# ucsdarclab/Python-SuPer

Hardware: AMD Instinct MI355X
Metric: LM iterations/s (embedded-deformation LM, point-to-plane + ARAP + Rot) (higher is better)
Workload: dtype f64; 1 GPU; C2: 200000 surfels / 2000 ED nodes / KNN=4, point-to-plane + ARAP + Rot, 10 LM iterations + Surfels.update per frame; frames_per_gpu=8, streams_per_gpu=1, global_frames=8, parallelism=frames sharded over 1 GPU(s), beta all-gather

## Files before the change

python-super_amd/csrc/slm_api.hip:

```cpp
#include <new>
#include <cstdio>

#include "slm_solver.h"

static thread_local std::string g_err;

void slm_set_error_text(const char* msg) { g_err = msg; }

std::atomic<long long> g_reallocs{0}, g_realloc_bytes{0}, g_plan_builds{0}, g_plan_reuses{0}, g_plan_fill_hits{0};

int check_slots(slm_solver* s, int first, int n) {
  if (!s) return fail(SLM_ERR_INVALID, "null solver");
  if (first < 0 || n < 1 || first + n > (int)s->slots.size())
    return fail(SLM_ERR_INVALID, "slot range out of bounds");
  for (int i = first; i < first + n; ++i) {
    join_prepare(s, i);
    if (!s->slots[i].h.bound) return fail(SLM_ERR_UNBOUND, "slot used before slm_bind_frame");
    if (s->slots[i].h.f.K != s->slots[first].h.f.K)
      return fail(SLM_ERR_UNSUPPORTED, "the frames of one batch must have the same num_neighbors");
  }
  return SLM_OK;
}

extern "C" {
// ... 120 lines not shown
  }
  return SLM_OK;
}

int slm_device_count(void) {
  int n = 0;
  if (hipGetDeviceCount(&n) != hipSuccess) return 0;
  return n;
}

int slm_create(const slm_config* cfg, slm_solver** out) {
  if (!cfg || !out) return fail(SLM_ERR_INVALID, "slm_create: null argument");
  if (cfg->max_frames < 1 || cfg->num_iterations < 0 || !(cfg->v > 0.0))
    return fail(SLM_ERR_INVALID, "slm_create: bad config");
  if (cfg->solver_path < 0 || cfg->solver_path > 4) return fail(SLM_ERR_INVALID, "slm_create: solver_path must be 0..4");
  if (cfg->data_path < 0 || cfg->data_path > 2) return fail(SLM_ERR_INVALID, "slm_create: data_path must be 0..2");
  if (slm_device_count() < 1) return fail(SLM_ERR_NO_DEVICE, "slm_create: no HIP device visible");
  slm_solver* s = new (std::nothrow) slm_solver();
  if (!s) return fail(SLM_ERR_HIP, "slm_create: out of host memory");
  s->cfg = *cfg;
  try {
    s->slots.resize(cfg->max_frames);
  } catch (...) {
    delete s;
    return fail(SLM_ERR_HIP, "slm_create: out of host memory");
  }
  const size_t n_slots = (size_t)cfg->max_frames;
  hipError_t e = s->frames_dev.grow(n_slots, n_slots);
  if (e == hipSuccess) e = hipMemset(s->frames_dev, 0, sizeof(FrameDev) * n_slots);
  if (e == hipSuccess) e = s->bw_dev.grow(2, 2);
  if (e == hipSuccess) e = s->reuse_dev.grow(n_slots, n_slots);
  if (e == hipSuccess) e = hipMemset(s->reuse_dev, 0, sizeof(int) * n_slots);
  if (e == hipSuccess) e = s->bw_host.grow(2, 2);
  if (e == hipSuccess) {
    s->prep = prep_create();
    if (!s->prep) e = hipErrorOutOfMemory;
  }
  if (e != hipSuccess) {
    g_err = std::string("slm_create: ") + hipGetErrorString(e);
    slm_destroy(s);
    return SLM_ERR_HIP;
  }
  {
    int dev = 0;
    (void)hipGetDevice(&dev);
    (void)dag_device_setup(dev, nullptr);
  }
  if (const char* hb = getenv("SLM_HYBRID")) s->hybrid_batches = atoi(hb) != 0;
  if (const char* dm = getenv("SLM_DAG_MAX_NODES")) s->dag_max_nodes = atol(dm);
  if (const char* nr = getenv("SLM_NO_REUSE")) s->no_reuse = atoi(nr) != 0;
  if (const char* pf = getenv("SLM_PURE_FILL")) s->pure_fill = atoi(pf) != 0;
  if (const char* fb = getenv("SLM_FUSE_BEGIN")) s->fuse_begin = atoi(fb) != 0;
  if (const char* gw = getenv("SLM_GRAM_WGS")) s->gram_wgs = std::min(std::max(atoi(gw), 0), 65535);
  {
    int dev = 0, cus = 0;
    (void)hipGetDevice(&dev);
    if (hipDeviceGetAttribute(&cus, hipDeviceAttributeMultiprocessorCount, dev) == hipSuccess && cus > 0) s->n_cus = cus;
  }
  *out = s;
  return SLM_OK;
}

int slm_destroy(slm_solver* s) {
  if (!s) return SLM_OK;
  s->prep_worker.shutdown();
  s->bind_pool.shutdown();
  for (Slot& sl : s->slots) {
    plan_free(sl.plan);
    pairplan_free(sl.pplan);
    if (sl.prep_fork) (void)hipEventDestroy(sl.prep_fork);
    if (sl.prep_done) (void)hipEventDestroy(sl.prep_done);
  }
  s->slots.clear();
  prep_destroy(s->prep);
  prep_destroy(s->prep_async);
  if (s->prep_stream) (void)hipStreamDestroy(s->prep_stream);
  for (PrepBuffers* pb : s->bind_prep) prep_destroy(pb);
  for (hipStream_t q : s->bind_streams) (void)hipStreamDestroy(q);
  for (hipEvent_t e : s->bind_events) (void)hipEventDestroy(e);
  for (auto& evs : s->ev_runs)
    for (hipEvent_t e : evs)
      if (e) (void)hipEventDestroy(e);
  for (hipEvent_t e : s->ev_pool) (void)hipEventDestroy(e);
  if (s->drain_event) (void)hipEventDestroy(s->drain_event);
  delete s;
  return SLM_OK;
}

int slm_get_plan_info(slm_solver* s, int32_t slot, double* out_caller, int32_t capacity) {
  int rc = check_slots(s, slot, 1);
  if (rc) return rc;
  if (!out_caller || capacity < 0) return fail(SLM_ERR_INVALID, "slm_get_plan_info: bad output");
  const Slot& sl = s->slots[slot];
  const FrameDev& h = sl.h;
  double out[SLM_PLAN_INFO_DOUBLES];
  for (int i = 0; i < SLM_PLAN_INFO_DOUBLES; ++i) out[i] = 0.0;
  if (h.nd_ready) {
    out[0] = 0.0;
    out[1] = (double)sl.cache.nd.fronts.size();
    out[2] = (double)sl.cache.nd.level_start.size() - 1.0;
    out[3] = sl.cache.nd.flops;
    out[10] = sl.cache.nd.flops_exact;
    out[11] = (double)sl.cache.nd.dag_tasks.size() / 2.0;
    out[4] = 8.0 * (double)sl.cache.nd.tile_doubles;
    out[12] = (double)sl.n_piv_tiles;
    out[13] = (double)sl.n_pure_tiles;
// ... 148 lines not shown
```

python-super_amd/csrc/slm_data.h:

```cpp
#pragma once
#include "slm_common.h"

#define SLM_KMAX 8
template <int KK>
struct SurfelEvalT {
  bool match;
  double r;
  int id[KK];
  double row[KK * 7];
  double c[3];
  int taps[4];
};
typedef SurfelEvalT<SLM_K> SurfelEval;

__device__ __forceinline__ void rows_from_c(const d3 p, const int id[4], const double w[4], double lam,
                                            const double* __restrict__ npk, const d3 c, double row[SLM_K * 7]) {
#pragma unroll
  for (int k = 0; k < 4; ++k) {
    const double2* nq = reinterpret_cast<const double2*>(npk + (size_t)SLM_NPK * id[k]);
    const double2 n0 = nq[0], n1 = nq[1], n3 = nq[3], n4 = nq[4];
    const d3 g = {n3.y, n4.x, n4.y};
    double jq[4];
    quat_jac_row(n0.x, {n0.y, n1.x, n1.y}, p - g, c, jq);
    const double lw = lam * w[k];
    row[7 * k + 0] = lw * jq[0];
    row[7 * k + 1] = lw * jq[1];
    row[7 * k + 2] = lw * jq[2];
    row[7 * k + 3] = lw * jq[3];
    row[7 * k + 4] = lw * c.x;
    row[7 * k + 5] = lw * c.y;
    row[7 * k + 6] = lw * c.z;
  }
}

template <int MODE, int KK, bool PX = false>
__device__ __forceinline__ void eval_surfel_coreT(const FrameDev& fd, const d3 p, const int id[KK], const double w[KK],
                                                  double lam, const double* __restrict__ npk, SurfelEvalT<KK>& out) {
  const FrameIn& f = frame_in(fd);

  double qw[KK];
  d3 qv[KK], dk[KK];
  d3 T = {0.0, 0.0, 0.0};
#pragma unroll
  for (int k = 0; k < KK; ++k) {
    out.id[k] = id[k];
    const double2* nq = reinterpret_cast<const double2*>(npk + (size_t)SLM_NPK * id[k]);
    const double2 n0 = nq[0], n1 = nq[1], n2 = nq[2], n3 = nq[3], n4 = nq[4];
    const double bb[7] = {n0.x, n0.y, n1.x, n1.y, n2.x, n2.y, n3.x};
    const d3 g = {n3.y, n4.x, n4.y};
    qw[k] = bb[0];
    qv[k] = {bb[1], bb[2], bb[3]};
    dk[k] = p - g;
    d3 t = quat_apply(qw[k], qv[k], dk[k]);
    t = {t.x + bb[4] + g.x, t.y + bb[5] + g.y, t.z + bb[6] + g.z};
    T = {T.x + w[k] * t.x, T.y + w[k] * t.y, T.z + w[k] * t.z};
  }

  out.match = false;
  out.r = 0.0;
  out.taps[0] = out.taps[1] = out.taps[2] = out.taps[3] = -1;

  const double fx = (double)f.fx, fy = (double)f.fy, cx = (double)f.cx, cy = (double)f.cy;
  const double Ze = T.z + 1e-8;
  const double u_ = T.x * fx / Ze + cx;
  const double v_ = T.y * fy / Ze + cy;
  const double ur = rint(u_), vr = rint(v_);
  const int H = f.H, W = f.W;
  const bool pv = vr >= 0.0 && vr < (double)(H - 1) && ur >= 0.0 && ur < (double)(W - 1);
  const double fv = floor(v_), cv = ceil(v_), fu = floor(u_), cu = ceil(u_);
  const double nn[4] = {fv, fv, cv, cv};
  const double mm[4] = {fu, cu, fu, cu};
  d3 o = {0, 0, 0}, n = {0, 0, 0};
  d3 dou = {0, 0, 0}, dov = {0, 0, 0}, dnu = {0, 0, 0}, dnv = {0, 0, 0};
  float4 tpv[4], tnv[4];
  if constexpr (PX) {
    bool all_ok = pv;
#pragma unroll
    for (int t = 0; t < 4; ++t) {
      const int ni = (int)nn[t], mi = (int)mm[t];
      const bool inside = pv && (ni >= 0) && (ni < H) && (mi >= 0) && (mi < W);
      const float4* q = fd.tgt_px.get() + 2 * (size_t)(inside ? ni * W + mi : 0);
      tpv[t] = q[0];
      tnv[t] = q[1];
      all_ok = all_ok && inside && tpv[t].w != 0.f;
    }
    const int tr = ((vr != fv) ? 2 : 0) + ((ur != fu) ? 1 : 0);
    const float tvf = tr == 0 ? tnv[0].w : (tr == 1 ? tnv[1].w : (tr == 2 ? tnv[2].w : tnv[3].w));
    if (!pv || tvf == 0.f) return;
    if (!all_ok) return;
  } else {
    const int coords = pv ? (int)vr * W + (int)ur : 0;
    const uint8_t tv = pv ? f.tgt_valid[coords] : (uint8_t)0;
    int rows[4];
#pragma unroll
    for (int t = 0; t < 4; ++t) {
      const int ni = (int)nn[t], mi = (int)mm[t];
      const bool inside = pv && (ni >= 0) && (ni < H) && (mi >= 0) && (mi < W);
      rows[t] = inside ? f.index_map[ni * W + mi] : -1;
    }
    if (!tv) return;
    bool all_ok = true;
#pragma unroll
    for (int t = 0; t < 4; ++t) {
      out.taps[t] = rows[t];
      all_ok = all_ok && (rows[t] >= 0);
    }
    if (!all_ok) return;
#pragma unroll
    for (int t = 0; t < 4; ++t) {
      tpv[t] = fd.tgt_pn[2 * (size_t)rows[t]];
      tnv[t] = fd.tgt_pn[2 * (size_t)rows[t] + 1];
    }
  }
#pragma unroll
  for (int t = 0; t < 4; ++t) {
    const double dn = nn[t] - v_, dm = mm[t] - u_;
    const double an = fmax(1.0 - fabs(dn), 0.0), am = fmax(1.0 - fabs(dm), 0.0);
    const float4 tp = tpv[t], tn = tnv[t];
    const d3 P = {(double)tp.x, (double)tp.y, (double)tp.z};
    const d3 Nn = {(double)tn.x, (double)tn.y, (double)tn.z};
    const double wv = an * am;
    o = {o.x + P.x * wv, o.y + P.y * wv, o.z + P.z * wv};
    n = {n.x + Nn.x * wv, n.y + Nn.y * wv, n.z + Nn.z * wv};
    if (MODE) {
      const double sn = dn >= 0.0 ? 1.0 : -1.0, sm = dm >= 0.0 ? 1.0 : -1.0;
      const double gu = an * sm, gv = am * sn;
      dou = {dou.x + P.x * gu, dou.y + P.y * gu, dou.z + P.z * gu};
      dov = {dov.x + P.x * gv, dov.y + P.y * gv, dov.z + P.z * gv};
      dnu = {dnu.x + Nn.x * gu, dnu.y + Nn.y * gu, dnu.z + Nn.z * gu};
      dnv = {dnv.x + Nn.x * gv, dnv.y + Nn.y * gv, dnv.z + Nn.z * gv};
    }
  }
  if (!(o.x == o.x && o.y == o.y && o.z == o.z && n.x == n.x && n.y == n.y && n.z == n.z)) return;

  const d3 e = T - o;
  out.match = true;
  out.r = lam * dot(n, e);
  if (!MODE) return;

  const double Z = T.z;
  const d3 Pi0 = {fx / Z, 0.0, -fx * T.x / (Z * Z)};
  const d3 Pi1 = {0.0, fy / Z, -fy * T.y / (Z * Z)};
  const double s0 = dot(e, dnu) - dot(n, dou);
  const double s1 = dot(e, dnv) - dot(n, dov);
  const d3 c = {n.x + s0 * Pi0.x + s1 * Pi1.x, n.y + s0 * Pi0.y + s1 * Pi1.y,
                n.z + s0 * Pi0.z + s1 * Pi1.z};
  out.c[0] = c.x;
  out.c[1] = c.y;
  out.c[2] = c.z;
  if (MODE == 2) return;
#pragma unroll
  for (int k = 0; k < KK; ++k) {
    double jq[4];
    quat_jac_row(qw[k], qv[k], dk[k], c, jq);
    const double lw = lam * w[k];
    out.row[7 * k + 0] = lw * jq[0];
    out.row[7 * k + 1] = lw * jq[1];
    out.row[7 * k + 2] = lw * jq[2];
    out.row[7 * k + 3] = lw * jq[3];
    out.row[7 * k + 4] = lw * c.x;
    out.row[7 * k + 5] = lw * c.y;
    out.row[7 * k + 6] = lw * c.z;
  }
}

template <int MODE, bool PX = false>
__device__ __forceinline__ void eval_surfel_core(const FrameDev& fd, const d3 p, int4 ids, const double w[4],
                                                 double lam, const double* __restrict__ npk, SurfelEval& out) {
  const int id[4] = {ids.x, ids.y, ids.z, ids.w};
  eval_surfel_coreT<MODE, SLM_K, PX>(fd, p, id, w, lam, npk, out);
}

template <int MODE>
__device__ __forceinline__ void eval_surfel_at(const FrameDev& fd, const void* __restrict__ sf_pts,
                                               const int* __restrict__ sf_idx,
                                               const void* __restrict__ sf_w, double lam,
                                               const double* __restrict__ npk, int i,
                                               SurfelEval& out) {
  double w[4];
  ld_state4(sf_w, (size_t)i, fd.f.state_f64, w);
  eval_surfel_core<MODE>(fd, ld_state3(sf_pts, (size_t)i, fd.f.state_f64),
                         *reinterpret_cast<const int4*>(sf_idx + 4 * (size_t)i), w, lam, npk, out);
}

template <int MODE, int KK>
__device__ __forceinline__ void eval_surfel(const FrameDev& fd, double lam, const double* npk, int i, SurfelEvalT<KK>& out) {
  const FrameIn& f = frame_in(fd);
  if constexpr (KK == SLM_K) {
    eval_surfel_at<MODE>(fd, f.sf_points, f.sf_knn_idx, f.sf_knn_w, lam, npk, i, out);
  } else {
    double wk[KK];
    int idk[KK];
    const void* wp = f.sf_knn_w;
#pragma unroll
    for (int k = 0; k < KK; ++k) {
      idk[k] = f.sf_knn_idx[(size_t)KK * i + k];
      wk[k] = fd.f.state_f64 ? static_cast<const double*>(wp)[(size_t)KK * i + k] : (double)static_cast<const float*>(wp)[(size_t)KK * i + k];
    }
    eval_surfel_coreT<MODE, KK>(fd, ld_state3(f.sf_points, (size_t)i, fd.f.state_f64), idk, wk, lam, npk, out);
// ... 3 lines not shown
```

python-super_amd/csrc/slm_data_k4.hip:

```cpp
#include <cstdlib>

#include "slm_data.h"
#include "slm_begin.h"
#include "slm_launch.h"

#define ROW_STRIDE 17

__global__ void __launch_bounds__(256) k_data_eval(const FrameDev* __restrict__ frames, double lam, int mode,
                                                    const int* __restrict__ reuse) {
  __shared__ double sm[16];
  __shared__ int s_skip;
  if (mode == 1 && reuse && reuse[blockIdx.y]) return;
  const FrameDev& fd = frames[blockIdx.y];
  if (!fd.bound || !fd.v1_ready || fd.st->stopped) return;
  if (mode == 1) {
    if (threadIdx.x == 0) s_skip = __hip_atomic_load(&fd.st->eval_valid, __ATOMIC_RELAXED, __HIP_MEMORY_SCOPE_AGENT) == 1;
    __syncthreads();
    if (s_skip) return;
  }
  const double* npk = mode == 0 ? fd.node_pk_try.get() : fd.node_pk.get();
  const int p0 = 256 * fd.wg_lo, p1 = min(fd.n_pos, 256 * fd.wg_hi);
  double acc = 0.0;
  int cnt = 0;
  for (int pos = p0 + blockIdx.x * blockDim.x + threadIdx.x; pos < p1; pos += gridDim.x * blockDim.x) {
    const int4 ids = *reinterpret_cast<const int4*>(fd.s_idx + 4 * (size_t)pos);
    double2 o0 = make_double2(0.0, 0.0), o1 = make_double2(0.0, 0.0);
    if (ids.x >= 0) {
      double wk[4];
      ld_state4(fd.s_w, (size_t)pos, fd.f.state_f64, wk);
      const d3 pp = ld_state3(fd.s_pts, (size_t)pos, fd.f.state_f64);
      SurfelEval ev;
      eval_surfel_core<2, true>(fd, pp, ids, wk, lam, npk, ev);
      if (ev.match) {
        acc += ev.r * ev.r;
        ++cnt;
        o0 = make_double2(ev.r, ev.c[0]);
        o1 = make_double2(ev.c[1], ev.c[2]);
      }
    }
    double2* out = reinterpret_cast<double2*>(fd.ev_rc.get() + 4 * (size_t)pos);
    out[0] = o0;
    out[1] = o1;
  }
  const double s = block_sum(acc, sm);
  const double c = block_sum((double)cnt, sm);
  if (threadIdx.x == 0) {
    fd.loss_part[2 * blockIdx.x] = s;
    fd.loss_part[2 * blockIdx.x + 1] = c;
    LMState* st = fd.st;
    const unsigned long long old = __hip_atomic_fetch_add(&st->eval_acc, (1ull << 32) | (unsigned long long)(unsigned)(int)c,
                                                          __ATOMIC_RELAXED, __HIP_MEMORY_SCOPE_AGENT);
    if ((int)(old >> 32) == (int)gridDim.x - 1) {
      st->m_eval = (int)(unsigned)(old & 0xFFFFFFFFull) + (int)c;
      __hip_atomic_store(&st->eval_acc, 0ull, __ATOMIC_RELAXED, __HIP_MEMORY_SCOPE_AGENT);
      if (mode != 0) __hip_atomic_store(&st->eval_valid, 1, __ATOMIC_RELAXED, __HIP_MEMORY_SCOPE_AGENT);
    }
  }
}

struct GramChunk {
  int my_run;
  int rec0, nrec;
  int4 ids;
  double2 e0, e1;
  double2 wa, wb;
  double px, py, pz;
  float4 wf;
  float qx, qy, qz;
};
template <bool MERGE>
__device__ __forceinline__ void gram_chunk_load(const FrameDev& fd, int c, int w, int l, int f64, GramChunk& k) {
  k.my_run = -1;
  k.rec0 = k.nrec = 0;
  k.ids = int4{-1, -1, -1, -1};
  k.e0 = k.e1 = k.wa = k.wb = make_double2(0.0, 0.0);
  k.px = k.py = k.pz = 0.0;
  k.wf = make_float4(0.f, 0.f, 0.f, 0.f);
  k.qx = k.qy = k.qz = 0.f;
  if (MERGE) {
    k.rec0 = fd.wg_first[c];
    k.nrec = fd.wg_last[c] - k.rec0 + 1;
  }
  const int base = (c * 4 + w) * 64;
  if (base >= fd.n_pos) return;
  const size_t pos = (size_t)(base + l);
  k.my_run = fd.grp_run[(base >> 2) + (l & 15)];
  const double2* e2 = reinterpret_cast<const double2*>(fd.ev_rc.get() + 4 * pos);
  k.e0 = e2[0];
  k.e1 = e2[1];
  k.ids = *reinterpret_cast<const int4*>(fd.s_idx + 4 * pos);
  if (f64) {
    const double2* q = reinterpret_cast<const double2*>(static_cast<const double*>(fd.s_w.get()) + 4 * pos);
    k.wa = q[0];
    k.wb = q[1];
    const double* pq = static_cast<const double*>(fd.s_pts.get()) + 3 * pos;
    k.px = pq[0]; k.py = pq[1]; k.pz = pq[2];
  } else {
    k.wf = *reinterpret_cast<const float4*>(static_cast<const float*>(fd.s_w.get()) + 4 * pos);
    const float* pq = static_cast<const float*>(fd.s_pts.get()) + 3 * pos;
    k.qx = pq[0]; k.qy = pq[1]; k.qz = pq[2];
  }
}
__device__ __forceinline__ void gram_lidx_load(const FrameDev& fd, int my_run, int l, uint8_t lv[3]) {
#pragma unroll
  for (int k = 0; k < 3; ++k) {
    const int idx = l + 64 * k;
// ... 218 lines not shown
  if (!fd.bound || !fd.v1_ready || fd.st->stopped) return;
  const int bi = blockIdx.x * 4 + (threadIdx.x >> 6);
  if (bi >= fd.n_blocks) return;
  const int l = threadIdx.x & 63;
  const unsigned key = (unsigned)fd.blk_key[bi];
  const int a = (int)(key / (unsigned)fd.f.J), b = (int)(key % (unsigned)fd.f.J);
  const int ca = l / 7, cb = l % 7;
  const bool act = (l < 49) && (a != b || ca >= cb);
  const bool jt = (a == b) && l >= 49 && l < 56;
  double acc = 0.0;
  if (fd.v2_ready) {
    const int s0 = fd.blk2_start[bi], s1 = fd.blk2_start[bi + 1];
    if (l < SLM_WREC)
      for (int s = s0; s < s1; ++s) acc += fd.wgslab[(size_t)fd.blk2_entry[s] * SLM_WREC + l];
  } else {
    const int s0 = fd.blk_start[bi], s1 = fd.blk_start[bi + 1];
    for (int s = s0; s < s1; ++s) {
      const int pl = fd.blk_entry[s];
      const int run = pl >> 4, pa = (pl >> 2) & 3, pb = pl & 3;
      const double* G = fd.slab + (size_t)run * SLM_SLAB_STRIDE;
      if (act) acc += gram_at(G, 7 * pa + ca, 7 * pb + cb);
      else if (jt) acc += gram_at(G, 28, 7 * pa + (l - 49));
    }
  }
  if (act) *band_entry(fd, 7 * a + ca, 7 * b + cb) = acc;
  else if (jt) fd.rhs[7 * a + (l - 49)] = -acc;
}

static int gram_wgs(int wgs, int n_frames, int n_cus) { return wgs > 0 ? wgs : max(1, 2 * n_cus / max(1, n_frames)); }

void launch_begin_and_gram(const FrameDev* frames_dev, int n_frames, double lam, hipStream_t st, const int* reuse,
                           int dag_cut, int wgs, int n_cus) {
  int dbg = 0;
#ifdef SLM_STAMPS
  if (const char* e = getenv("SLM_DBG")) dbg = atoi(e);
#endif
  hipLaunchKernelGGL((k_data_gram<true, true>), dim3(gram_wgs(wgs, n_frames, n_cus), n_frames), dim3(256), 0, st, frames_dev, lam, dbg,
                     reuse, dag_cut);
}

void launch_data_gram(const FrameDev* frames_dev, int n_frames, int max_pos, double lam, int variants,
                      hipStream_t st, const int* reuse, int wgs, int n_cus) {
  if (max_pos <= 0) return;
  int dbg = 0;
#ifdef SLM_STAMPS
  if (const char* e = getenv("SLM_DBG")) dbg = atoi(e);
#endif
  const dim3 grid(wgs > 0 ? wgs : min(gram_wgs(0, n_frames, n_cus), (max_pos + 255) / 256), n_frames);
  if (variants & 1) hipLaunchKernelGGL(k_data_gram<true>, grid, dim3(256), 0, st, frames_dev, lam, dbg, reuse, -2);
  if (variants & 2) hipLaunchKernelGGL(k_data_gram<false>, grid, dim3(256), 0, st, frames_dev, lam, dbg, reuse, -2);
}

void launch_data_eval(const FrameDev* frames_dev, int n_frames, int n_blocks, double lam, int mode, hipStream_t st,
                      const int* reuse) {
  hipLaunchKernelGGL(k_data_eval, dim3(n_blocks, n_frames), dim3(256), 0, st, frames_dev, lam, mode, reuse);
}

void launch_band_assemble(const FrameDev* frames_dev, int n_frames, int max_blocks, hipStream_t st) {
  if (max_blocks <= 0) return;
  hipLaunchKernelGGL(k_band_assemble, dim3((max_blocks + 3) / 4, n_frames), dim3(256), 0, st, frames_dev);
}
```

python-super_amd/csrc/slm_launch.h:

```cpp
#pragma once
#include "slm_common.h"

void launch_data_grad(const FrameDev*, int, int, int, double, hipStream_t);
void launch_data_grad_pairs(const FrameDev*, int, int, int, double, hipStream_t);
void launch_data_loss(const FrameDev*, int, int, int, double, int, hipStream_t);
void launch_data_resid(const FrameDev*, int, int, int, double, double*, uint8_t*, int32_t*, hipStream_t);

void launch_data_gram(const FrameDev*, int, int, double, int, hipStream_t, const int* reuse, int wgs, int n_cus);
void launch_begin_and_gram(const FrameDev*, int, double, hipStream_t, const int* reuse, int dag_cut, int wgs, int n_cus);
void launch_data_eval(const FrameDev*, int, int, double, int mode, hipStream_t, const int* reuse = nullptr);
void launch_band_assemble(const FrameDev*, int, int, hipStream_t);

void launch_front_assemble(const FrameDev*, int, int, hipStream_t);
void launch_pair_reduce(const FrameDev*, int, int, hipStream_t);
void launch_pair_scatter(const FrameDev*, int, int, hipStream_t);
void launch_reg_grad_nd(const FrameDev*, int, int, int, double, int, double, hipStream_t);
void launch_front_load_rhs(const FrameDev*, int, int, hipStream_t);
void launch_iter_begin_nd(const FrameDev*, int, hipStream_t, const int* reuse, int dag_cut);
void launch_front_solve(const FrameDev*, int, const NDLevelSched*, int, double, hipStream_t);
void launch_front_levels(const FrameDev*, int, const NDLevelSched*, int, int, int, double, hipStream_t);

bool ensure_dynamic_lds(const void* kernel, size_t bytes);

int launch_front_solve_dag(const FrameDev*, int, int, double, hipStream_t, int cut, bool reset, bool check);
int dag_device_setup(int dev, int* xcd8_out);
int dag_last_mode();
hipError_t set_dag_timeout_ticks(long long);
void launch_dag_abort_check(const FrameDev*, int, hipStream_t);

void launch_bandwidth(const slm_frame&, int*, hipStream_t);
void launch_band_solve(const FrameDev*, int, int, int, double, hipStream_t);
void launch_band_to_dense(const FrameDev*, int, double*, hipStream_t);
void launch_dense_to_band(const FrameDev*, const double*, const double*, hipStream_t);

void launch_reg_grad(const FrameDev*, int, int, int, double, int, double, hipStream_t);
void launch_after_solve(const FrameDev*, int, int, int, int, double, int, double, int, hipStream_t);
void launch_reg_loss(const FrameDev*, int, int, int, double, int, double, int, hipStream_t);

void launch_init_slot(const FrameDev*, int, int, const slm_config&, hipStream_t);
void launch_iter_begin(const FrameDev*, int, hipStream_t);
void launch_pack_nodes(const FrameDev*, int, int, hipStream_t);
void launch_make_trial(const FrameDev*, int, int, hipStream_t);
void launch_pack_target(int, const float*, const float*, float4*, hipStream_t);
void launch_pack_target_px(int, const int*, const uint8_t*, const float*, const float*, float4*, hipStream_t);
void launch_accept(const FrameDev*, int, int, int, int, hipStream_t, int* reuse = nullptr, int eval_pass = 0);
void launch_loss_out(const FrameDev*, int, int, double*, hipStream_t);
void launch_zero_reg_part(const FrameDev*, int, int, hipStream_t);
```

python-super_amd/csrc/slm_lm.hip:

```cpp
#include "slm_solver.h"

namespace {
struct BatchDims {
  int maxN = 0, maxJKe = 0, nt_max = 0, wb_cap = 0, n_reg_part = 0;
  int max_pos = 0, max_blocks = 0, maxP = 0;
  bool corr = false;
  int n_acc_part = 0;
  int K = 0;
  int gram_variants = 0;
  bool nd = true;
  DataForm form = DataForm::none;
  const int* reuse = nullptr;
  bool fused_begin = false;
  int* accept_reuse = nullptr;
  int accept_eval = 0;
  int max_tasks = 0;
  int hybrid_cut = -2, hybrid_levels = -1, max_top_tasks = 0;
  std::vector<NDLevelSched> sched;
};
BatchDims dims_of(slm_solver* s, int first, int n, bool band = false) {
  BatchDims d;
  bool all_v1 = true, all_vk = true;
  for (int i = first; i < first + n; ++i) {
    const FrameDev& h = s->slots[i].h;
// ... 58 lines not shown
    if (m.first < 0) m.schur_at = m.pull_at = -1;
    if (m.schur_at == -2) m.schur_at = -1;
    if (m.pull_at == -2) m.pull_at = -1;
  }
  if (s->cfg.use_arap || s->cfg.use_rot)
    d.n_reg_part = std::min(kRegBlocksMax, (d.maxJKe + 255) / 256);
  d.n_acc_part = d.n_reg_part + (s->corr_mode ? kCorrBlocks : 0);
  return d;
}
}

bool solve_is_task_graph(const slm_solver* s, int n, int J) {
  return s->cfg.solver_path == 2 || (s->cfg.solver_path == 0 && (n <= 2 || (long)n * J <= s->dag_max_nodes));
}

namespace {
static bool solve_is_hybrid(const slm_solver* s, int n, const BatchDims& d) {
  return !solve_is_task_graph(s, n, d.maxP / 7) && (s->cfg.solver_path == 4 || (s->cfg.solver_path == 0 && s->hybrid_batches)) &&
         d.hybrid_cut >= 0 && d.hybrid_levels == (int)d.sched.size() && d.hybrid_cut + 1 < d.hybrid_levels;
}
static int dag_cut_of(const slm_solver* s, int n, const BatchDims& d) {
  if (solve_is_task_graph(s, n, d.maxP / 7)) return -1;
  return solve_is_hybrid(s, n, d) ? d.hybrid_cut : -2;
}
int enqueue_front_solve(slm_solver* s, const FrameDev* fr, int n, const BatchDims& d, double u_override, hipStream_t st,
                        bool dag_reset_done = false, bool dag_check_later = false) {
  const bool dag = solve_is_task_graph(s, n, d.maxP / 7);
  const bool hybrid = solve_is_hybrid(s, n, d);
  s->last_solver_form = dag ? 1 : (hybrid ? 2 : 0);
  int mode = -1;
  if (dag) {
    mode = launch_front_solve_dag(fr, n, d.max_tasks, u_override, st, -1, !dag_reset_done, !dag_check_later);
  } else if (hybrid) {
    const int n_levels = (int)d.sched.size(), l_cut = n_levels - 1 - d.hybrid_cut;
    launch_front_levels(fr, n, d.sched.data(), n_levels, l_cut, 0, u_override, st);
    mode = launch_front_solve_dag(fr, n, d.max_top_tasks, u_override, st, d.hybrid_cut, !dag_reset_done, !dag_check_later);
  } else {
    launch_front_solve(fr, n, d.sched.data(), (int)d.sched.size(), u_override, st);
  }
  s->last_dag_mode = mode;
  return mode;
}

void enqueue_zero(const FrameDev* fr, int n, const BatchDims& d, hipStream_t st, const int* reuse, int dag_cut, bool fused) {
  if (!d.nd) launch_iter_begin(fr, n, st);
  else if (!fused) launch_iter_begin_nd(fr, n, st, reuse, dag_cut);
}

void enqueue_jacobian(slm_solver* s, const FrameDev* fr, int n, const BatchDims& d, hipStream_t st, int eval_mode,
                      const int* reuse, int dag_cut, bool fused) {
  const double w = s->cfg.w_data;
  switch (d.form) {
    case DataForm::tuple:
      if (eval_mode >= 0) launch_data_eval(fr, n, kLossBlocks, w, eval_mode, st, reuse);
      if (fused) launch_begin_and_gram(fr, n, w, st, reuse, dag_cut, s->gram_wgs, s->n_cus);
      else launch_data_gram(fr, n, d.max_pos, w, d.gram_variants, st, reuse, s->gram_wgs, s->n_cus);
      break;
    case DataForm::pairs:
      launch_data_grad_pairs(fr, n, d.maxN, d.K, w, st);
      if (d.corr) launch_corr_grad_pairs(fr, s->corr_dev + (fr - s->frames_dev), n, d.maxN, d.K, s->corr_mode, s->corr_w, st);
      break;
    case DataForm::per_entry:
      launch_data_grad(fr, n, d.maxN, d.K, w, st);
      if (d.corr) launch_corr_grad(fr, s->corr_dev + (fr - s->frames_dev), n, d.maxN, d.K, s->corr_mode, s->corr_w, st);
      break;
    case DataForm::none: break;
  }
}

enum class Shard { whole, before_exchange, after_exchange };
void enqueue_scatter(slm_solver* s, const FrameDev* fr, int n, const BatchDims& d, hipStream_t st, Shard part) {
  const slm_config& c = s->cfg;
  const bool tuple = d.form == DataForm::tuple;
  if (part == Shard::before_exchange) {
    if (tuple) launch_pair_reduce(fr, n, d.max_blocks, st);
    return;
  }
  if (part == Shard::after_exchange || d.form == DataForm::pairs) launch_pair_scatter(fr, n, d.max_blocks, st);
  else if (tuple && d.nd) launch_front_assemble(fr, n, d.max_blocks, st);
  else if (tuple) launch_band_assemble(fr, n, d.max_blocks, st);
  if (d.nd) {
    launch_reg_grad_nd(fr, n, d.maxP / 7, c.use_arap, c.w_arap, c.use_rot, c.w_rot, st);
    if (!c.use_arap && !c.use_rot) launch_front_load_rhs(fr, n, d.maxP, st);
  } else {
    launch_reg_grad(fr, n, d.maxJKe, c.use_arap, c.w_arap, c.use_rot, c.w_rot, st);
  }
}

void enqueue_data_loss(slm_solver* s, const FrameDev* fr, int n, const BatchDims& d, hipStream_t st, bool at_beta) {
  if (d.form == DataForm::tuple && !at_beta) launch_data_eval(fr, n, kLossBlocks, s->cfg.w_data, 0, st);
  else if (d.form != DataForm::none) launch_data_loss(fr, n, kLossBlocks, d.K, s->cfg.w_data, at_beta ? 0 : 1, st);
  if (s->corr_mode && d.K >= 1)
    launch_corr_loss(fr, s->corr_dev + (fr - s->frames_dev), n, d.K, s->corr_mode, s->corr_w, at_beta ? 0 : 1, 2 * d.n_reg_part,
                     kCorrCntPart, st);
}
}

extern "C" {

static hipEvent_t take_event(slm_solver* s) {
  if (!s->ev_pool.empty()) {
    hipEvent_t e = s->ev_pool.back();
    s->ev_pool.pop_back();
    return e;
  }
  hipEvent_t e = nullptr;
  if (hipEventCreate(&e) != hipSuccess) return nullptr;
  return e;
}

int slm_set_shard(slm_solver* s, int32_t rank, int32_t world) {
  if (!s || world < 1 || rank < 0 || rank >= world) return fail(SLM_ERR_INVALID, "slm_set_shard: bad rank/world");
  if (s->cfg.data_path != 0 || s->cfg.solver_path == 1)
    return fail(SLM_ERR_UNSUPPORTED, "slm_set_shard: needs data_path 0 and a nested-dissection solver_path (0, 2, 3 or 4)");
  if (s->corr_mode)
    return fail(SLM_ERR_UNSUPPORTED, "slm_set_shard: the correspondence term is enabled (slm_enable_corr); it needs every surfel of "
                                     "the frame on one device");
  s->rank = rank;
  s->world = world;
  s->shard_mode = true;
  for (size_t i = 0; i < s->slots.size(); ++i) {
    join_prepare(s, (int)i);
    s->slots[i].model_ready = false;
    s->slots[i].h.bound = 0;
  }
  HIPCHK(hipMemset(s->frames_dev, 0, sizeof(FrameDev) * s->slots.size()));
  return SLM_OK;
}

static int shard_dims(slm_solver* s, int n_frames, BatchDims& d) {
  int rc = check_slots(s, 0, n_frames);
  if (rc) return rc;
  d = dims_of(s, 0, n_frames);
  if (!d.nd || (d.form != DataForm::tuple && d.form != DataForm::pairs))
    return fail(SLM_ERR_UNSUPPORTED, "sharded LM step: every slot needs a multifrontal data path (tuple-sorted or K-generic) and the ND solver");
  return SLM_OK;
}

int slm_lm_grad_local(slm_solver* s, int32_t n_frames, void* stream) {
  BatchDims d;
  int rc = shard_dims(s, n_frames, d);
  if (rc) return rc;
  hipStream_t st = (hipStream_t)stream;
// ... 335 lines not shown
```

python-super_amd/csrc/slm_solver.h:

```cpp
#pragma once
#include <algorithm>
#include <atomic>
#include <mutex>
#include <string>
#include <vector>

#include "slm_common.h"
#include "slm_corr.h"
#include "slm_host.h"
#include "slm_launch.h"
#include "slm_prep.h"
#include "slm_workers.h"

constexpr int kLossBlocks = 512;
constexpr int kRegBlocksMax = 64;
constexpr int kCorrBlocks = SLM_CORR_BLOCKS;
constexpr int kCorrCntPart = 2 * (kRegBlocksMax + kCorrBlocks);
constexpr size_t kLossPartDoubles = (size_t)2 * (kLossBlocks + kRegBlocksMax + kCorrBlocks) + kCorrBlocks;

enum class DataForm {
  none,
  tuple,
  pairs,
  per_entry,
// ... 24 lines not shown
  DevBuf<uint8_t> corr_valid;
  PairPlan pplan;
  PlanCache cache;
  DevBuf<NDDest> d_cur_dests;
  PinnedBuf<uint32_t> h_pairs;
  PinnedBuf<int32_t> h_knn;
  PinnedBuf<float> h_pts;
  PinnedBuf<double> h_pts64;
  PinnedBuf<FrameDev> h_pin;
  DevBuf<NDFront> d_fronts;
  DevBuf<NDTileItem> d_items;
  DevBuf<uint8_t> d_tile_kind;
  DevBuf<long long> d_zero_tiles;
  int n_piv_tiles = 0, n_pure_tiles = 0;
  int prep_kind = 0, prep_max_bin = 0;
  std::vector<uint8_t> h_tile_kind;
  std::vector<long long> h_zero_tiles;
  DevBuf<int32_t> d_ints;
  DevBuf<long long> d_dag_trace;
  DevBuf<int32_t> d_dag_flags;
  DevBuf<NDDest> d_dests;
  DevBuf<double> ftiles, fvec, flinv, fmail;
  DevBuf<double> pairbuf;
  DevBuf<double> band, linv;
  bool band_ready = false;
  bool model_ready = false;
  slm_frame prep_model{};
  unsigned long long prep_ticket = 0;
  int prep_rc = SLM_OK;
  bool prep_recorded = false;
  std::string prep_err;
  hipEvent_t prep_fork = nullptr, prep_done = nullptr;
};

struct slm_solver {
  PrepBuffers* prep = nullptr;
  BindPool bind_pool;
  AsyncWorker prep_worker;
  PrepBuffers* prep_async = nullptr;
  hipStream_t prep_stream = nullptr;
  std::vector<PrepBuffers*> bind_prep;
  std::vector<hipStream_t> bind_streams;
  std::vector<hipEvent_t> bind_events;
  std::mutex band_mutex;
  hipEvent_t drain_event = nullptr;
  double drain_est_ms = 0.0;
  int last_solver_form = -1;
  int last_dag_mode = -1;
  bool no_reuse = false;
  bool hybrid_batches = true;
  long dag_max_nodes = 8000;
  bool fuse_begin = true;
  int gram_wgs = 0;
  int n_cus = 256;
  bool pure_fill = true;
  bool profile = false;
  std::vector<hipEvent_t> ev_pool;
  std::vector<std::vector<hipEvent_t>> ev_runs;
  slm_config cfg{};
  std::vector<Slot> slots;
  DevBuf<FrameDev> frames_dev;
  DevBuf<int> bw_dev;
  PinnedBuf<int> bw_host;
  DevBuf<int> reuse_dev;
  int rank = 0, world = 1;
  int corr_mode = 0;
  double corr_w = 0.0;
  DevBuf<CorrDev> corr_dev;
  bool shard_mode = false;
};

extern std::atomic<long long> g_reallocs, g_realloc_bytes, g_plan_builds, g_plan_reuses, g_plan_fill_hits;

template <typename T>
hipError_t grow(DevBuf<T>& b, size_t need) {
  if (need <= b.cap) return hipSuccess;
  const size_t want = need + need / 8;
  ++g_reallocs;
  g_realloc_bytes += (long long)(want * sizeof(T));
  return b.grow(need, want);
}

#pragma GCC visibility push(hidden)
int check_slots(slm_solver* s, int first, int n);
void join_prepare(slm_solver* s, int slot);
int ensure_band(slm_solver* s, int slot, hipStream_t st);
bool solve_is_task_graph(const slm_solver* s, int n, int J);
#pragma GCC visibility pop
```

Baseline: 3379 LM it/s.

## Software-pipeline data eval kernel with persistent workgroups and prefetched node/tap loads

Splits the per-surfel evaluation into load, skin/project, tap-fetch and residual stages, and rewrites k_data_eval as a persistent kernel. Each workgroup walks a contiguous set of virtual blocks and pipelines three items: it prefetches node parameters and state for the next surfel and the pixel taps for the current one while finishing the previous residual. The grid is sized to a waves-per-EU target times the CU count instead of a fixed 512 blocks, with per-virtual-block wave sums kept in shared memory so loss_part keeps its layout. The aim is to hide gather latency, at the cost of more registers, extra shared memory and more complex block partitioning.

Result: no change. 3398 LM it/s (median of 6 runs) (+0.6%).

```diff
diff --git a/python-super_amd/csrc/slm_api.hip b/python-super_amd/csrc/slm_api.hip
--- a/python-super_amd/csrc/slm_api.hip
+++ b/python-super_amd/csrc/slm_api.hip
@@ -196,6 +196,7 @@
   if (const char* pf = getenv("SLM_PURE_FILL")) s->pure_fill = atoi(pf) != 0;
   if (const char* fb = getenv("SLM_FUSE_BEGIN")) s->fuse_begin = atoi(fb) != 0;
   if (const char* gw = getenv("SLM_GRAM_WGS")) s->gram_wgs = std::min(std::max(atoi(gw), 0), 65535);
+  if (const char* ew = getenv("SLM_EVAL_WGS")) s->eval_wgs = std::min(std::max(atoi(ew), 0), 65535);
   {
     int dev = 0, cus = 0;
     (void)hipGetDevice(&dev);
diff --git a/python-super_amd/csrc/slm_data.h b/python-super_amd/csrc/slm_data.h
--- a/python-super_amd/csrc/slm_data.h
+++ b/python-super_amd/csrc/slm_data.h
@@ -33,19 +33,27 @@
   }
 }
 
-template <int MODE, int KK, bool PX = false>
-__device__ __forceinline__ void eval_surfel_coreT(const FrameDev& fd, const d3 p, const int id[KK], const double w[KK],
-                                                  double lam, const double* __restrict__ npk, SurfelEvalT<KK>& out) {
-  const FrameIn& f = frame_in(fd);
-
-  double qw[KK];
-  d3 qv[KK], dk[KK];
+
+template <int KK>
+struct EvalNodesT {
+  double2 n[KK][5];
+};
+template <int KK>
+__device__ __forceinline__ void eval_nodes_load(const double* __restrict__ npk, const int id[KK], EvalNodesT<KK>& nd) {
+#pragma unroll
+  for (int k = 0; k < KK; ++k) {
+    const double2* nq = reinterpret_cast<const double2*>(npk + (size_t)SLM_NPK * id[k]);
+    nd.n[k][0] = nq[0]; nd.n[k][1] = nq[1]; nd.n[k][2] = nq[2]; nd.n[k][3] = nq[3]; nd.n[k][4] = nq[4];
+  }
+}
+
+template <int KK>
+__device__ __forceinline__ d3 eval_skin(const EvalNodesT<KK>& nd, const d3 p, const double w[KK], double qw[KK], d3 qv[KK],
+                                        d3 dk[KK]) {
   d3 T = {0.0, 0.0, 0.0};
 #pragma unroll
   for (int k = 0; k < KK; ++k) {
-    out.id[k] = id[k];
-    const double2* nq = reinterpret_cast<const double2*>(npk + (size_t)SLM_NPK * id[k]);
-    const double2 n0 = nq[0], n1 = nq[1], n2 = nq[2], n3 = nq[3], n4 = nq[4];
+    const double2 n0 = nd.n[k][0], n1 = nd.n[k][1], n2 = nd.n[k][2], n3 = nd.n[k][3], n4 = nd.n[k][4];
     const double bb[7] = {n0.x, n0.y, n1.x, n1.y, n2.x, n2.y, n3.x};
     const d3 g = {n3.y, n4.x, n4.y};
     qw[k] = bb[0];
@@ -55,63 +63,77 @@
     t = {t.x + bb[4] + g.x, t.y + bb[5] + g.y, t.z + bb[6] + g.z};
     T = {T.x + w[k] * t.x, T.y + w[k] * t.y, T.z + w[k] * t.z};
   }
-
-  out.match = false;
-  out.r = 0.0;
-  out.taps[0] = out.taps[1] = out.taps[2] = out.taps[3] = -1;
-
+  return T;
+}
+
+struct EvalProj {
+  double u_, v_;
+  bool pv;
+};
+struct EvalCell {
+  double ur, vr, fu, cu, fv, cv;
+};
+__device__ __forceinline__ EvalCell eval_cell(const EvalProj& pr) {
+  EvalCell c;
+  c.ur = rint(pr.u_); c.vr = rint(pr.v_);
+  c.fv = floor(pr.v_); c.cv = ceil(pr.v_); c.fu = floor(pr.u_); c.cu = ceil(pr.u_);
+  return c;
+}
+__device__ __forceinline__ EvalProj eval_project(const FrameIn& f, const d3 T) {
   const double fx = (double)f.fx, fy = (double)f.fy, cx = (double)f.cx, cy = (double)f.cy;
   const double Ze = T.z + 1e-8;
-  const double u_ = T.x * fx / Ze + cx;
-  const double v_ = T.y * fy / Ze + cy;
-  const double ur = rint(u_), vr = rint(v_);
+  EvalProj pr;
+  pr.u_ = T.x * fx / Ze + cx;
+  pr.v_ = T.y * fy / Ze + cy;
+  const double ur = rint(pr.u_), vr = rint(pr.v_);
+  pr.pv = vr >= 0.0 && vr < (double)(f.H - 1) && ur >= 0.0 && ur < (double)(f.W - 1);
+  return pr;
+}
+
+__device__ __forceinline__ void eval_taps_px(const FrameDev& fd, const FrameIn& f, const EvalProj& pr, float4 tpv[4],
+                                             float4 tnv[4]) {
+  const EvalCell cl = eval_cell(pr);
+  const double nn[4] = {cl.fv, cl.fv, cl.cv, cl.cv};
+  const double mm[4] = {cl.fu, cl.cu, cl.fu, cl.cu};
   const int H = f.H, W = f.W;
-  const bool pv = vr >= 0.0 && vr < (double)(H - 1) && ur >= 0.0 && ur < (double)(W - 1);
-  const double fv = floor(v_), cv = ceil(v_), fu = floor(u_), cu = ceil(u_);
-  const double nn[4] = {fv, fv, cv, cv};
-  const double mm[4] = {fu, cu, fu, cu};
+#pragma unroll
+  for (int t = 0; t < 4; ++t) {
+    const int ni = (int)nn[t], mi = (int)mm[t];
+    const bool inside = pr.pv && (ni >= 0) && (ni < H) && (mi >= 0) && (mi < W);
+    const float4* q = fd.tgt_px.get() + 2 * (size_t)(inside ? ni * W + mi : 0);
+    tpv[t] = q[0];
+    tnv[t] = q[1];
+  }
+}
+__device__ __forceinline__ bool eval_match_px(const FrameIn& f, const EvalProj& pr, const float4 tpv[4], const float4 tnv[4]) {
+  const EvalCell cl = eval_cell(pr);
+  const double nn[4] = {cl.fv, cl.fv, cl.cv, cl.cv};
+  const double mm[4] = {cl.fu, cl.cu, cl.fu, cl.cu};
+  const int H = f.H, W = f.W;
+  bool all_ok = pr.pv;
+#pragma unroll
+  for (int t = 0; t < 4; ++t) {
+    const int ni = (int)nn[t], mi = (int)mm[t];
+    const bool inside = pr.pv && (ni >= 0) && (ni < H) && (mi >= 0) && (mi < W);
+    all_ok = all_ok && inside && tpv[t].w != 0.f;
+  }
+  const bool hi_v = cl.vr != cl.fv, hi_u = cl.ur != cl.fu;
+  const bool z0 = tnv[0].w == 0.f, z1 = tnv[1].w == 0.f, z2 = tnv[2].w == 0.f, z3 = tnv[3].w == 0.f;
+  const bool tv_zero = (!hi_v & !hi_u & z0) | (!hi_v & hi_u & z1) | (hi_v & !hi_u & z2) | (hi_v & hi_u & z3);
+  if (!pr.pv || tv_zero) return false;
+  return all_ok;
+}
+
+template <int MODE>
+__device__ __forceinline__ bool eval_residual(const FrameIn& f, const d3 T, const EvalProj& pr, const float4 tpv[4],
+                                              const float4 tnv[4], double lam, double& r, d3& c) {
+  const double fx = (double)f.fx, fy = (double)f.fy;
+  const double u_ = pr.u_, v_ = pr.v_;
+  const EvalCell cl = eval_cell(pr);
+  const double nn[4] = {cl.fv, cl.fv, cl.cv, cl.cv};
+  const double mm[4] = {cl.fu, cl.cu, cl.fu, cl.cu};
   d3 o = {0, 0, 0}, n = {0, 0, 0};
   d3 dou = {0, 0, 0}, dov = {0, 0, 0}, dnu = {0, 0, 0}, dnv = {0, 0, 0};
-  float4 tpv[4], tnv[4];
-  if constexpr (PX) {
-    bool all_ok = pv;
-#pragma unroll
-    for (int t = 0; t < 4; ++t) {
-      const int ni = (int)nn[t], mi = (int)mm[t];
-      const bool inside = pv && (ni >= 0) && (ni < H) && (mi >= 0) && (mi < W);
-      const float4* q = fd.tgt_px.get() + 2 * (size_t)(inside ? ni * W + mi : 0);
-      tpv[t] = q[0];
-      tnv[t] = q[1];
-      all_ok = all_ok && inside && tpv[t].w != 0.f;
-    }
-    const int tr = ((vr != fv) ? 2 : 0) + ((ur != fu) ? 1 : 0);
-    const float tvf = tr == 0 ? tnv[0].w : (tr == 1 ? tnv[1].w : (tr == 2 ? tnv[2].w : tnv[3].w));
-    if (!pv || tvf == 0.f) return;
-    if (!all_ok) return;
-  } else {
-    const int coords = pv ? (int)vr * W + (int)ur : 0;
-    const uint8_t tv = pv ? f.tgt_valid[coords] : (uint8_t)0;
-    int rows[4];
-#pragma unroll
-    for (int t = 0; t < 4; ++t) {
-      const int ni = (int)nn[t], mi = (int)mm[t];
-      const bool inside = pv && (ni >= 0) && (ni < H) && (mi >= 0) && (mi < W);
-      rows[t] = inside ? f.index_map[ni * W + mi] : -1;
-    }
-    if (!tv) return;
-    bool all_ok = true;
-#pragma unroll
-    for (int t = 0; t < 4; ++t) {
-      out.taps[t] = rows[t];
-      all_ok = all_ok && (rows[t] >= 0);
-    }
-    if (!all_ok) return;
-#pragma unroll
-    for (int t = 0; t < 4; ++t) {
-      tpv[t] = fd.tgt_pn[2 * (size_t)rows[t]];
-      tnv[t] = fd.tgt_pn[2 * (size_t)rows[t] + 1];
-    }
-  }
 #pragma unroll
   for (int t = 0; t < 4; ++t) {
     const double dn = nn[t] - v_, dm = mm[t] - u_;
@@ -131,20 +153,77 @@
       dnv = {dnv.x + Nn.x * gv, dnv.y + Nn.y * gv, dnv.z + Nn.z * gv};
     }
   }
-  if (!(o.x == o.x && o.y == o.y && o.z == o.z && n.x == n.x && n.y == n.y && n.z == n.z)) return;
+  if (!(o.x == o.x && o.y == o.y && o.z == o.z && n.x == n.x && n.y == n.y && n.z == n.z)) return false;
 
   const d3 e = T - o;
-  out.match = true;
-  out.r = lam * dot(n, e);
-  if (!MODE) return;
+  r = lam * dot(n, e);
+  if (!MODE) return true;
 
   const double Z = T.z;
   const d3 Pi0 = {fx / Z, 0.0, -fx * T.x / (Z * Z)};
   const d3 Pi1 = {0.0, fy / Z, -fy * T.y / (Z * Z)};
   const double s0 = dot(e, dnu) - dot(n, dou);
   const double s1 = dot(e, dnv) - dot(n, dov);
-  const d3 c = {n.x + s0 * Pi0.x + s1 * Pi1.x, n.y + s0 * Pi0.y + s1 * Pi1.y,
-                n.z + s0 * Pi0.z + s1 * Pi1.z};
+  c = {n.x + s0 * Pi0.x + s1 * Pi1.x, n.y + s0 * Pi0.y + s1 * Pi1.y, n.z + s0 * Pi0.z + s1 * Pi1.z};
+  return true;
+}
+
+template <int MODE, int KK, bool PX = false>
+__device__ __forceinline__ void eval_surfel_coreT(const FrameDev& fd, const d3 p, const int id[KK], const double w[KK],
+                                                  double lam, const double* __restrict__ npk, SurfelEvalT<KK>& out) {
+  const FrameIn& f = frame_in(fd);
+
+  double qw[KK];
+  d3 qv[KK], dk[KK];
+#pragma unroll
+  for (int k = 0; k < KK; ++k) out.id[k] = id[k];
+  EvalNodesT<KK> nd;
+  eval_nodes_load<KK>(npk, id, nd);
+  const d3 T = eval_skin<KK>(nd, p, w, qw, qv, dk);
+
+  out.match = false;
+  out.r = 0.0;
+  out.taps[0] = out.taps[1] = out.taps[2] = out.taps[3] = -1;
+
+  const EvalProj pr = eval_project(f, T);
+  float4 tpv[4], tnv[4];
+  if constexpr (PX) {
+    eval_taps_px(fd, f, pr, tpv, tnv);
+    if (!eval_match_px(f, pr, tpv, tnv)) return;
+  } else {
+    const EvalCell cl = eval_cell(pr);
+    const double nn[4] = {cl.fv, cl.fv, cl.cv, cl.cv};
+    const double mm[4] = {cl.fu, cl.cu, cl.fu, cl.cu};
+    const int H = f.H, W = f.W;
+    const int coords = pr.pv ? (int)cl.vr * W + (int)cl.ur : 0;
+    const uint8_t tv = pr.pv ? f.tgt_valid[coords] : (uint8_t)0;
+    int rows[4];
+#pragma unroll
+    for (int t = 0; t < 4; ++t) {
+      const int ni = (int)nn[t], mi = (int)mm[t];
+      const bool inside = pr.pv && (ni >= 0) && (ni < H) && (mi >= 0) && (mi < W);
+      rows[t] = inside ? f.index_map[ni * W + mi] : -1;
+    }
+    if (!tv) return;
+    bool all_ok = true;
+#pragma unroll
+    for (int t = 0; t < 4; ++t) {
+      out.taps[t] = rows[t];
+      all_ok = all_ok && (rows[t] >= 0);
+    }
+    if (!all_ok) return;
+#pragma unroll
+    for (int t = 0; t < 4; ++t) {
+      tpv[t] = fd.tgt_pn[2 * (size_t)rows[t]];
+      tnv[t] = fd.tgt_pn[2 * (size_t)rows[t] + 1];
+    }
+  }
+  double r = 0.0;
+  d3 c = {0.0, 0.0, 0.0};
+  if (!eval_residual<MODE>(f, T, pr, tpv, tnv, lam, r, c)) return;
+  out.match = true;
+  out.r = r;
+  if (!MODE) return;
   out.c[0] = c.x;
   out.c[1] = c.y;
   out.c[2] = c.z;
diff --git a/python-super_amd/csrc/slm_data_k4.hip b/python-super_amd/csrc/slm_data_k4.hip
--- a/python-super_amd/csrc/slm_data_k4.hip
+++ b/python-super_amd/csrc/slm_data_k4.hip
@@ -6,9 +6,70 @@
 
 #define ROW_STRIDE 17
 
-__global__ void __launch_bounds__(256) k_data_eval(const FrameDev* __restrict__ frames, double lam, int mode,
-                                                    const int* __restrict__ reuse) {
-  __shared__ double sm[16];
+struct EvalItem {
+  int pos;
+  int blk;
+  bool last;
+  int4 ids;
+};
+struct EvalState {
+  double2 wa, wb;
+  double px, py, pz;
+  float4 wf;
+  float qx, qy, qz;
+};
+struct EvalPending {
+  int pos, blk;
+  bool has, live, last;
+  d3 T;
+  EvalProj pr;
+  float4 tpv[4], tnv[4];
+};
+__device__ __forceinline__ void eval_state_load(const FrameDev& fd, size_t pos, int f64, EvalState& k) {
+  k.wa = k.wb = make_double2(0.0, 0.0);
+  k.px = k.py = k.pz = 0.0;
+  k.wf = make_float4(0.f, 0.f, 0.f, 0.f);
+  k.qx = k.qy = k.qz = 0.f;
+  if (f64) {
+    const double2* q = reinterpret_cast<const double2*>(static_cast<const double*>(fd.s_w.get()) + 4 * pos);
+    k.wa = q[0];
+    k.wb = q[1];
+    const double* pq = static_cast<const double*>(fd.s_pts.get()) + 3 * pos;
+    k.px = pq[0]; k.py = pq[1]; k.pz = pq[2];
+  } else {
+    k.wf = *reinterpret_cast<const float4*>(static_cast<const float*>(fd.s_w.get()) + 4 * pos);
+    const float* pq = static_cast<const float*>(fd.s_pts.get()) + 3 * pos;
+    k.qx = pq[0]; k.qy = pq[1]; k.qz = pq[2];
+  }
+}
+__device__ __forceinline__ d3 eval_state_get(const EvalState& k, int f64, double wk[4]) {
+  if (f64) {
+    wk[0] = k.wa.x; wk[1] = k.wa.y; wk[2] = k.wb.x; wk[3] = k.wb.y;
+    return {k.px, k.py, k.pz};
+  }
+  wk[0] = (double)k.wf.x; wk[1] = (double)k.wf.y; wk[2] = (double)k.wf.z; wk[3] = (double)k.wf.w;
+  return {(double)k.qx, (double)k.qy, (double)k.qz};
+}
+
+__device__ __forceinline__ int eval_first_block(int w, int nwg, int q, int rm, int n_vb) {
+  const int nlive = q > 0 ? n_vb : rm;
+  const int t = (int)(((long long)q * n_vb + rm) * w / nwg);
+  int b;
+  if (t <= (q + 1) * rm) b = (t + q) / (q + 1);
+  else b = rm + (t - (q + 1) * rm + q - 1) / q;
+  return min(b, nlive);
+}
+
+#define SLM_EVAL_VB_MAX 512
+#ifndef SLM_EVAL_WAVES
+#define SLM_EVAL_WAVES 2
+#endif
+
+__global__ void __launch_bounds__(256) __attribute__((amdgpu_waves_per_eu(SLM_EVAL_WAVES, SLM_EVAL_WAVES)))
+k_data_eval(const FrameDev* __restrict__ frames, double lam, int mode, const int* __restrict__ reuse, int n_vb) {
+  __shared__ double w_sum[SLM_EVAL_VB_MAX][4];
+  __shared__ int w_cnt[SLM_EVAL_VB_MAX][4];
+  __shared__ int s_cnt;
   __shared__ int s_skip;
   if (mode == 1 && reuse && reuse[blockIdx.y]) return;
   const FrameDev& fd = frames[blockIdx.y];
@@ -18,40 +79,145 @@
     __syncthreads();
     if (s_skip) return;
   }
+  if (threadIdx.x == 0) s_cnt = 0;
+  const FrameIn& f = frame_in(fd);
+  const int f64 = fd.f.state_f64;
   const double* npk = mode == 0 ? fd.node_pk_try.get() : fd.node_pk.get();
   const int p0 = 256 * fd.wg_lo, p1 = min(fd.n_pos, 256 * fd.wg_hi);
+  const int nch = p1 > p0 ? (p1 - p0 + 255) >> 8 : 0;
+  const int q = nch / n_vb, rm = nch - q * n_vb;
+  const int nlive = q > 0 ? n_vb : rm;
+  const int w = blockIdx.x, nwg = gridDim.x;
+  const int bl0 = eval_first_block(w, nwg, q, rm, n_vb), bl1 = eval_first_block(w + 1, nwg, q, rm, n_vb);
+  const int wv = threadIdx.x >> 6, lane = threadIdx.x & 63;
+
+  int nb = bl0, nk = 0;
+  auto fetch = [&](EvalItem& it) __attribute__((always_inline)) {
+    it.pos = it.blk = -1;
+    it.last = false;
+    if (nb < bl1) {
+      const int pos = p0 + 256 * nb + (int)threadIdx.x + nk * 256 * n_vb;
+      it.pos = pos < p1 ? pos : -1;
+      it.blk = nb;
+      ++nk;
+      it.last = nk >= q + (nb < rm ? 1 : 0);
+      if (it.last) {
+        ++nb;
+        nk = 0;
+      }
+    }
+    it.ids = *reinterpret_cast<const int4*>(fd.s_idx + 4 * (size_t)(it.pos >= 0 ? it.pos : p0));
+  };
+  const int n_items = (q * bl1 + min(bl1, rm)) - (q * bl0 + min(bl0, rm));
+
   double acc = 0.0;
   int cnt = 0;
-  for (int pos = p0 + blockIdx.x * blockDim.x + threadIdx.x; pos < p1; pos += gridDim.x * blockDim.x) {
-    const int4 ids = *reinterpret_cast<const int4*>(fd.s_idx + 4 * (size_t)pos);
-    double2 o0 = make_double2(0.0, 0.0), o1 = make_double2(0.0, 0.0);
-    if (ids.x >= 0) {
-      double wk[4];
-      ld_state4(fd.s_w, (size_t)pos, fd.f.state_f64, wk);
-      const d3 pp = ld_state3(fd.s_pts, (size_t)pos, fd.f.state_f64);
-      SurfelEval ev;
-      eval_surfel_core<2, true>(fd, pp, ids, wk, lam, npk, ev);
-      if (ev.match) {
-        acc += ev.r * ev.r;
-        ++cnt;
-        o0 = make_double2(ev.r, ev.c[0]);
-        o1 = make_double2(ev.c[1], ev.c[2]);
+  EvalItem A, N, N2;
+  EvalPending C;
+  C.has = C.live = C.last = false;
+  C.pos = C.blk = -1;
+  C.T = {0.0, 0.0, 0.0};
+  C.pr.u_ = C.pr.v_ = 0.0;
+  C.pr.pv = false;
+  if (n_items > 0) {
+    fetch(A);
+    fetch(N);
+    bool liveA = A.pos >= 0 && A.ids.x >= 0;
+    bool liveN = N.pos >= 0 && N.ids.x >= 0;
+    int idN[4] = {liveN ? N.ids.x : 0, liveN ? N.ids.y : 0, liveN ? N.ids.z : 0, liveN ? N.ids.w : 0};
+    EvalNodesT<SLM_K> nd;
+    EvalState sa;
+    {
+      const int idA[4] = {liveA ? A.ids.x : 0, liveA ? A.ids.y : 0, liveA ? A.ids.z : 0, liveA ? A.ids.w : 0};
+      eval_nodes_load<SLM_K>(npk, idA, nd);
+      eval_state_load(fd, (size_t)(A.pos >= 0 ? A.pos : p0), f64, sa);
+    }
+    eval_taps_px(fd, f, C.pr, C.tpv, C.tnv);
+#pragma unroll 1
+    for (int i = 0; i <= n_items; ++i) {
+      fetch(N2);
+      d3 T = {0.0, 0.0, 0.0};
+      EvalProj pr;
+      pr.u_ = pr.v_ = 0.0;
+      pr.pv = false;
+      if (liveA) {
+        double wk[4], qw[SLM_K];
+        d3 qv[SLM_K], dk[SLM_K];
+        const d3 pp = eval_state_get(sa, f64, wk);
+        T = eval_skin<SLM_K>(nd, pp, wk, qw, qv, dk);
+        pr = eval_project(f, T);
       }
-    }
-    double2* out = reinterpret_cast<double2*>(fd.ev_rc.get() + 4 * (size_t)pos);
-    out[0] = o0;
-    out[1] = o1;
-  }
-  const double s = block_sum(acc, sm);
-  const double c = block_sum((double)cnt, sm);
+      eval_nodes_load<SLM_K>(npk, idN, nd);
+      eval_state_load(fd, (size_t)(N.pos >= 0 ? N.pos : p0), f64, sa);
+      if (C.has) {
+        double2 o0 = make_double2(0.0, 0.0), o1 = make_double2(0.0, 0.0);
+        if (C.live && eval_match_px(f, C.pr, C.tpv, C.tnv)) {
+          double r = 0.0;
+          d3 c = {0.0, 0.0, 0.0};
+          if (eval_residual<2>(f, C.T, C.pr, C.tpv, C.tnv, lam, r, c)) {
+            acc += r * r;
+            ++cnt;
+            o0 = make_double2(r, c.x);
+            o1 = make_double2(c.y, c.z);
+          }
+        }
+        if (C.pos >= 0) {
+          double2* out = reinterpret_cast<double2*>(fd.ev_rc.get() + 4 * (size_t)C.pos);
+          out[0] = o0;
+          out[1] = o1;
+        }
+        if (C.last) {
+          const double s = wave_sum(acc);
+          const double c = wave_sum((double)cnt);
+          if (lane == 0) {
+            w_sum[C.blk - bl0][wv] = s;
+            w_cnt[C.blk - bl0][wv] = (int)c;
+          }
+          acc = 0.0;
+          cnt = 0;
+        }
+      }
+      C.pos = A.pos;
+      C.blk = A.blk;
+      C.has = i < n_items;
+      C.live = liveA;
+      C.last = A.last;
+      C.T = T;
+      C.pr = pr;
+      eval_taps_px(fd, f, pr, C.tpv, C.tnv);
+      A = N;
+      liveA = liveN;
+      N = N2;
+      liveN = N.pos >= 0 && N.ids.x >= 0;
+      idN[0] = liveN ? N.ids.x : 0; idN[1] = liveN ? N.ids.y : 0; idN[2] = liveN ? N.ids.z : 0; idN[3] = liveN ? N.ids.w : 0;
+    }
+  }
+  __syncthreads();
+  int mine = 0;
+  for (int j = threadIdx.x; j < bl1 - bl0; j += 256) {
+    double s = 0.0, c = 0.0;
+    for (int k = 0; k < 4; ++k) {
+      s += w_sum[j][k];
+      c += (double)w_cnt[j][k];
+    }
+    fd.loss_part[2 * (bl0 + j)] = s;
+    fd.loss_part[2 * (bl0 + j) + 1] = c;
+    mine += (int)c;
+  }
+  const int z0 = nlive + (int)((long long)(n_vb - nlive) * w / nwg), z1 = nlive + (int)((long long)(n_vb - nlive) * (w + 1) / nwg);
+  for (int j = z0 + threadIdx.x; j < z1; j += 256) {
+    fd.loss_part[2 * j] = 0.0;
+    fd.loss_part[2 * j + 1] = 0.0;
+  }
+  if (mine) atomicAdd(&s_cnt, mine);
+  __syncthreads();
   if (threadIdx.x == 0) {
-    fd.loss_part[2 * blockIdx.x] = s;
-    fd.loss_part[2 * blockIdx.x + 1] = c;
+    const int c = s_cnt;
     LMState* st = fd.st;
-    const unsigned long long old = __hip_atomic_fetch_add(&st->eval_acc, (1ull << 32) | (unsigned long long)(unsigned)(int)c,
+    const unsigned long long old = __hip_atomic_fetch_add(&st->eval_acc, (1ull << 32) | (unsigned long long)(unsigned)c,
                                                           __ATOMIC_RELAXED, __HIP_MEMORY_SCOPE_AGENT);
     if ((int)(old >> 32) == (int)gridDim.x - 1) {
-      st->m_eval = (int)(unsigned)(old & 0xFFFFFFFFull) + (int)c;
+      st->m_eval = (int)(unsigned)(old & 0xFFFFFFFFull) + c;
       __hip_atomic_store(&st->eval_acc, 0ull, __ATOMIC_RELAXED, __HIP_MEMORY_SCOPE_AGENT);
       if (mode != 0) __hip_atomic_store(&st->eval_valid, 1, __ATOMIC_RELAXED, __HIP_MEMORY_SCOPE_AGENT);
     }
@@ -376,8 +542,10 @@
 }
 
 void launch_data_eval(const FrameDev* frames_dev, int n_frames, int n_blocks, double lam, int mode, hipStream_t st,
-                      const int* reuse) {
-  hipLaunchKernelGGL(k_data_eval, dim3(n_blocks, n_frames), dim3(256), 0, st, frames_dev, lam, mode, reuse);
+                      int wgs, int n_cus, const int* reuse) {
+  n_blocks = min(n_blocks, SLM_EVAL_VB_MAX);
+  const int nwg = wgs > 0 ? wgs : min(n_blocks, max(1, SLM_EVAL_WAVES * n_cus / max(1, n_frames)));
+  hipLaunchKernelGGL(k_data_eval, dim3(nwg, n_frames), dim3(256), 0, st, frames_dev, lam, mode, reuse, n_blocks);
 }
 
 void launch_band_assemble(const FrameDev* frames_dev, int n_frames, int max_blocks, hipStream_t st) {
diff --git a/python-super_amd/csrc/slm_launch.h b/python-super_amd/csrc/slm_launch.h
--- a/python-super_amd/csrc/slm_launch.h
+++ b/python-super_amd/csrc/slm_launch.h
@@ -8,7 +8,7 @@
 
 void launch_data_gram(const FrameDev*, int, int, double, int, hipStream_t, const int* reuse, int wgs, int n_cus);
 void launch_begin_and_gram(const FrameDev*, int, double, hipStream_t, const int* reuse, int dag_cut, int wgs, int n_cus);
-void launch_data_eval(const FrameDev*, int, int, double, int mode, hipStream_t, const int* reuse = nullptr);
+void launch_data_eval(const FrameDev*, int, int, double, int mode, hipStream_t, int wgs, int n_cus, const int* reuse = nullptr);
 void launch_band_assemble(const FrameDev*, int, int, hipStream_t);
 
 void launch_front_assemble(const FrameDev*, int, int, hipStream_t);
diff --git a/python-super_amd/csrc/slm_lm.hip b/python-super_amd/csrc/slm_lm.hip
--- a/python-super_amd/csrc/slm_lm.hip
+++ b/python-super_amd/csrc/slm_lm.hip
@@ -134,7 +134,7 @@
   const double w = s->cfg.w_data;
   switch (d.form) {
     case DataForm::tuple:
-      if (eval_mode >= 0) launch_data_eval(fr, n, kLossBlocks, w, eval_mode, st, reuse);
+      if (eval_mode >= 0) launch_data_eval(fr, n, kLossBlocks, w, eval_mode, st, s->eval_wgs, s->n_cus, reuse);
       if (fused) launch_begin_and_gram(fr, n, w, st, reuse, dag_cut, s->gram_wgs, s->n_cus);
       else launch_data_gram(fr, n, d.max_pos, w, d.gram_variants, st, reuse, s->gram_wgs, s->n_cus);
       break;
@@ -170,7 +170,7 @@
 }
 
 void enqueue_data_loss(slm_solver* s, const FrameDev* fr, int n, const BatchDims& d, hipStream_t st, bool at_beta) {
-  if (d.form == DataForm::tuple && !at_beta) launch_data_eval(fr, n, kLossBlocks, s->cfg.w_data, 0, st);
+  if (d.form == DataForm::tuple && !at_beta) launch_data_eval(fr, n, kLossBlocks, s->cfg.w_data, 0, st, s->eval_wgs, s->n_cus);
   else if (d.form != DataForm::none) launch_data_loss(fr, n, kLossBlocks, d.K, s->cfg.w_data, at_beta ? 0 : 1, st);
   if (s->corr_mode && d.K >= 1)
     launch_corr_loss(fr, s->corr_dev + (fr - s->frames_dev), n, d.K, s->corr_mode, s->corr_w, at_beta ? 0 : 1, 2 * d.n_reg_part,
diff --git a/python-super_amd/csrc/slm_solver.h b/python-super_amd/csrc/slm_solver.h
--- a/python-super_amd/csrc/slm_solver.h
+++ b/python-super_amd/csrc/slm_solver.h
@@ -100,6 +100,7 @@
   long dag_max_nodes = 8000;
   bool fuse_begin = true;
   int gram_wgs = 0;
+  int eval_wgs = 0;
   int n_cus = 256;
   bool pure_fill = true;
   bool profile = false;
```
